# MartinPippel/DAmar

Hardware: AMD Instinct MI355X
Metric: aligned base-pairs/sec (daligner block-vs-block) (higher is better)
Workload: dtype int32

## Files before the change

### damar_amd/api.py

```python
import ctypes as C
import os

from .lib import load, bin_path

c_int64 = C.c_int64


class HITS_READ(C.Structure):
    _fields_ = [("rlen", C.c_int), ("boff", c_int64), ("coff", c_int64), ("flags", C.c_int)]


class HITS_DB(C.Structure):
    _fields_ = [("ureads", C.c_int), ("freq", C.c_float * 4), ("maxlen", C.c_int),
                ("totlen", c_int64), ("nreads", C.c_int), ("part", C.c_int), ("ufirst", C.c_int),
                ("path", C.c_char_p), ("loaded", C.c_int), ("bases", C.c_void_p),
                ("reads", C.POINTER(HITS_READ)), ("tracks", C.c_void_p)]


class SimParams(C.Structure):
    _fields_ = [("genome_mbp", C.c_double), ("coverage", C.c_double), ("bias", C.c_double),
                ("seed", C.c_int), ("rmean", C.c_int), ("rsdev", C.c_int), ("rshort", C.c_int),
                ("erate", C.c_double), ("block_mbp", C.c_int), ("min_len", C.c_int),
                ("tandem_frac", C.c_double), ("max_blocks", C.c_int)]

# ... 94 lines not shown
        L.damar_index_bytes.argtypes = [C.c_void_p]
        L.damar_index_bytes.restype = C.c_uint64
        L.damar_complement_copy.argtypes = [C.POINTER(HITS_DB), C.POINTER(HITS_DB)]
        L.damar_free_complement.argtypes = [C.POINTER(HITS_DB)]
        L.damar_async_drain.argtypes = []
        L.damar_set_bread_range.argtypes = [C.c_int, C.c_int]
        L.damar_index_download.argtypes = [C.c_void_p, C.c_void_p]
        L.damar_match.argtypes = [C.POINTER(HITS_DB), C.POINTER(HITS_DB), C.c_void_p, C.c_void_p,
                                  C.c_int, C.c_int, C.c_void_p, C.POINTER(c_int64)]
        L.damar_match_batch.argtypes = [C.POINTER(MatchJob), C.c_int]
        L.damar_set_async.argtypes = [C.c_int]
        L.damar_async_totals.argtypes = [C.POINTER(c_int64), C.POINTER(C.c_double), C.POINTER(C.c_double)]
        L.damar_async_counts.argtypes = [C.POINTER(c_int64), C.POINTER(C.c_double), C.POINTER(c_int64)]
        L.damar_wave_totals.argtypes = [C.POINTER(c_int64)] * 3
        L.damar_write_overlaps.argtypes = [C.c_void_p, C.c_char_p, C.c_char_p, C.c_char_p, C.c_char_p, C.c_int]
        L.damar_tandem_set_params.argtypes = [C.c_int] * 4
        L.damar_tandem_set_params.restype = C.c_int
        L.Match_Self.argtypes = [C.c_char_p, C.POINTER(HITS_DB), C.c_void_p]
        L.damar_match_self.argtypes = [C.POINTER(HITS_DB), C.c_void_p, C.c_void_p, C.POINTER(c_int64)]
        L.damar_last_seeds.argtypes = [C.c_void_p, c_int64]
        L.damar_last_seeds.restype = c_int64
        L.damar_order_runs_test.argtypes = [C.c_void_p, c_int64, C.c_int, C.c_int, C.c_void_p, C.c_int]
        L.damar_order_runs_test.restype = C.c_int
        L.damar_local_alignment_batch.argtypes = [C.c_void_p, C.c_void_p, C.c_int, C.c_void_p,
                                                  C.POINTER(C.c_int), C.c_int, C.POINTER(C.c_int),
                                                  C.POINTER(c_int64), C.POINTER(C.c_uint16), c_int64]
        L.damar_local_alignment_batch.restype = C.c_int
        L.damar_local_alignment_batch_opts.argtypes = L.damar_local_alignment_batch.argtypes + [C.c_int, C.POINTER(C.c_int),
                                                                                               C.POINTER(C.c_int)]
        L.damar_local_alignment_batch_opts.restype = C.c_int
        L.damar_last_timings.argtypes = [C.POINTER(C.c_double)]
        L.damar_last_counters.argtypes = [C.POINTER(c_int64)]
        L.damar_last_slabs.argtypes = [C.POINTER(C.c_int), C.POINTER(c_int64), C.c_int]
        L.damar_last_slabs.restype = C.c_int
        L.damar_slab_totals.argtypes = [C.POINTER(c_int64)]
        L.damar_slab_cut.argtypes = [C.POINTER(C.c_uint64), C.c_int, C.c_uint64, C.POINTER(C.c_int), C.POINTER(c_int64), C.c_int]
        L.damar_slab_cut.restype = C.c_int
        L.damar_bench_sort_u32.argtypes = [C.c_uint32, C.c_int, C.c_int, C.c_uint32]
        L.damar_bench_sort_u32.restype = C.c_double
        L.damar_set_check.argtypes = [C.c_int]
        L.damar_check_totals.argtypes = [C.POINTER(c_int64)]
        L.damar_check_note_blocks.argtypes = [C.c_void_p, C.POINTER(HITS_DB), C.POINTER(HITS_DB)]
        L.damar_pile_coverage.argtypes = [C.POINTER(PileBatch), C.POINTER(RepeatParams), C.POINTER(c_int64), C.POINTER(c_int64), C.POINTER(c_int64)]
        L.damar_pile_repeats.argtypes = [C.POINTER(PileBatch), C.POINTER(RepeatParams), C.POINTER(PileTrack)]
        L.damar_pile_tandem.argtypes = [C.POINTER(PileBatch), C.c_int, C.POINTER(PileTrack)]
        L.damar_pile_last.argtypes = [C.POINTER(C.c_double), C.POINTER(c_int64)]
# ... 444 lines not shown
```

### damar_amd/csrc/kernels/kernels.h

```cpp
#ifndef DAMAR_KERNELS_H
#define DAMAR_KERNELS_H

#include "dev_common.h"

size_t damar_scan_workspace_bytes(u64 n);
void   damar_exclusive_scan_u32(const u32 *in, u32 *out, u64 n, void *work, u64 *total_dev, hipStream_t st);
#define DAMAR_SCAN_TILE 4096
void   damar_tile_offsets_u32(const u32 *in, u64 n, void *work, u64 *total_dev, hipStream_t st);
void   damar_scan_tile_counts(u32 *tcount, u32 ntiles, u64 *total_dev, hipStream_t st);
size_t damar_sort_workspace_bytes(u64 n);
void   damar_sort_set_threads(int threads);
const u32 *damar_sort_error_word(const void *work);
int    damar_radix_sort_keys_u64(u64 *k0, u64 *k1, u64 n, int lobit, int hibit, void *work, hipStream_t st);
void   damar_radix_sort_split_u64(u64 *k0, u64 *k1, u64 n, int lobit, int hibit, u32 *ohi, u32 *olo, void *work,
                                  hipStream_t st);
int    damar_radix_sort_u32(u32 *k0, u32 *v0, u32 *k1, u32 *v1, u64 n, int nbits, void *work, hipStream_t st);
int    damar_radix_sort_keys_u32(u32 *k0, u32 *k1, u64 n, int nbits, void *work, hipStream_t st);
int    damar_radix_sort_u64(u64 *k0, u32 *v0, u64 *k1, u32 *v1, u64 n, int nbits, void *work, hipStream_t st);

enum { DAMAR_PILE_COVER = 0, DAMAR_PILE_REPEAT = 1, DAMAR_PILE_TANDEM = 2 };
#define DAMAR_PILE_ERR_RANGE 1u
typedef struct
{
  const long long *pile_off;
  const int *pile_aread, *abpos, *aepos, *bbpos, *bepos, *bread, *flags, *read_len, *read_flags;
  u32   npiles;
  int   mode, pbits;
  int   min_len, inc_identity, inccov, enter, leave, merge_dist;
  u64  *keys;
  u32  *kept;
  const u32 *koff;
// ... 131 lines not shown
} MergeArgs;

typedef struct { u32 b0, b1, ja, ia;
                 u32 sh, pad[3]; } MergeTile;

size_t damar_merge_workspace_bytes(u32 alen);
u32   *damar_merge_tile_counts(void *work, u32 alen);
u32    damar_merge_tiles(u32 alen);
void   damar_launch_merge_count(const MergeArgs *m, void *work, unsigned long long *gram, u32 ngram, hipStream_t st);
void damar_launch_merge_emit(const MergeArgs *m, void *work, u64 nhits, u64 *keys, u32 *vals, u32 *pid, hipStream_t st);
void damar_launch_merge_bread_hist(const MergeArgs *m, void *work, unsigned long long *hist, hipStream_t st);
void damar_launch_merge_range(const MergeArgs *m, void *work, hipStream_t st);
void damar_launch_pair_heads_ids(const u32 *pids, u64 nhits, u64 off, u64 gtotal, int abits, int minhit, int nshift,
                                 u64 *send, u64 *bits, void *scan_work, u64 *total_dev, u32 *heads, hipStream_t st);
void damar_launch_pair_bitmap(const u32 *pids, const u32 *heads, u32 nheads, int abits, u32 b_lo, u32 b_hi, u32 *bitmap,
                              hipStream_t st);
void damar_launch_seed_cut_count(const u64 *keys, u64 nhits, int pbits, const u32 *bitmap, u32 *tcount, u64 *total_dev,
                                 hipStream_t st);
void damar_launch_seed_cut_scatter(const u64 *keys, const u32 *vals, u64 nhits, int pbits, const u32 *bitmap,
                                   const u32 *toff, u64 *okeys, u32 *ovals, hipStream_t st);
void damar_launch_pair_heads(const u64 *keys, u64 nhits, u64 off, u64 gtotal, int pbits, int abits, int minhit, int nshift,
                             u64 *send , u64 *bits, void *scan_work, u64 *total_dev,
                             u32 *heads, hipStream_t st);
void damar_launch_pair_work(u64 *keys, const u32 *vals, u64 nhits, u64 off, u64 gtotal, int ppos, int dbits, int abits, int minhit, int nshift,
                            u64 *send , u64 *bits, void *scan_work, u64 *total_dev ,
                            int binshift, int kmer, int hitmin, u32 b_lo, u32 b_hi, int unsorted, hipStream_t st);
size_t damar_order_runs_scratch_bytes(u64 nhits);
void damar_launch_order_runs(u64 *keys, u64 nhits, int ppos, int dbits, const u32 *work, u32 nwork, void *scratch, hipStream_t st);
void damar_launch_pair_work_expand(const u64 *bits, const void *scan_work, u64 nhits, u32 *work, hipStream_t st);
#define WORK_COST_BITS 16
#define WORK_COST_MAX  ((1u << WORK_COST_BITS) - 1)
void damar_launch_work_cost(const u64 *keys, const u32 *vals, u64 nhits, int pbits, int abits, int dbits, const u32 *aboff,
                            const u32 *bboff, const u32 *work, u32 nwork, u32 coarse, u32 *key, u32 *val, hipStream_t st);
void damar_launch_pair_screen(const u64 *keys, const u32 *vals, u64 nhits, int pbits, int dbits, const u32 *heads, u32 nheads,
                              int minhit, int binshift, int kmer, int hitmin, int abits, u32 b_lo, u32 b_hi, u32 *keep, hipStream_t st);
void damar_launch_compact_u32(const u32 *src, const u32 *keep, const u32 *off, u32 n, u32 *out, hipStream_t st);
void damar_launch_compact_index(const u32 *flags, const u32 *off, u64 n, u32 *out, hipStream_t st);

#ifdef __HIPCC__
__device__ __forceinline__ int seed_diag(u64 k, const u32 *__restrict__ vals, u64 i, u64 pmask, int dbits)
{ if (dbits)
    return (int) ((k >> dbits) & pmask) - (int) (k & ((1ull << dbits) - 1));
  return (int) vals[i];
}
#endif

typedef struct
{ int abpos, bbpos, aepos, bepos, diffs;
  int atlen, btlen;
  int aread, bread;
  u32 item, seq;
  u32 toff;
// ... 147 lines not shown
```

### damar_amd/csrc/kernels/seed_merge.hip

```cpp
#include "dev_common.h"
#include "kernels.h"

SEED_PRIO_VAR(g_merge_prio, 0)
SEED_PRIO_SETTER(damar_merge_set_prio, g_merge_prio)


__device__ __forceinline__ u32 count_below(const u32 *__restrict__ bpos, u32 jb, u32 ib, u32 bound)
{ u32 a = jb, b = ib;
  while (a < b)
    { u32 m = (a + b) >> 1;
      if (bpos[m] < bound) a = m + 1; else b = m;
    }
  return a - jb;
}


#ifndef MT_PER
#define MT_PER  4
#endif
#define MT_A    (MT_PER * 256)
#define MT_BCAP (3 * MT_A)
#define MT_HITS 4
#define MT_NBK  2048

// ... 838 lines not shown
}

void damar_launch_merge_bread_hist(const MergeArgs *m, void *work, unsigned long long *hist, hipStream_t st)
{ if (m->alen == 0)
    return;
  const u32 ntiles = (u32) mw_tiles(m->alen);
  const u32 *cnt = (const u32 *) ((char *) work + mw_off_cnt(m->alen)), *jb = (const u32 *) ((char *) work + mw_off_jb(m->alen));
  hipLaunchKernelGGL(merge_bread_hist, dim3(ntiles), dim3(256), 0, st, *m, (const MergeTile *) work, cnt, jb, hist);
}

void damar_launch_merge_range(const MergeArgs *m, void *work, hipStream_t st)
{ if (m->alen == 0)
    return;
  const u32 ntiles = (u32) mw_tiles(m->alen);
  u32 *tcount = damar_merge_tile_counts(work, m->alen);
  u32 *cnt = (u32 *) ((char *) work + mw_off_cnt(m->alen)), *jb = (u32 *) ((char *) work + mw_off_jb(m->alen));
  hipLaunchKernelGGL(merge_range, dim3(ntiles), dim3(256), 0, st, *m, (const MergeTile *) work, tcount, cnt, jb);
}

#define SCREEN_MAX   48
#define SCREEN_PANEL 50000
template <typename K>
__global__ __launch_bounds__(64)
void slice_ends(const K *__restrict__ keys, u64 nhits, u64 off, u64 gtotal, int bshift, int nshift, u64 *__restrict__ send)
{ const int nthr = 1 << nshift, t = threadIdx.x;
  if (t >= nthr)
    return;
  const u64 g = (t == nthr - 1) ? gtotal : (gtotal * (u64) (t + 1)) >> nshift;
  u64 e;
  if (g <= off)
    e = 0;
  else if (g > off + nhits)
    e = ~0ull;
  else
    { e = g - off;
      u64 d = keys[e - 1] >> bshift, a = e, b = nhits;
      while (a < b)
        { u64 mid = (a + b) >> 1;
          if ((keys[mid] >> bshift) == d) a = mid + 1; else b = mid;
        }
      e = a;
    }
  send[t] = e;
}

#define PH_ROUNDS (DAMAR_SCAN_TILE / 256)
template <typename K>
__global__ __launch_bounds__(256)
// ... 43 lines not shown
                    for (int t = 0; t < nthr; t++)
                      { u64 e = send[t];
                        if (i < e)
                          { if (i + (u64) minhit >= e) f = false;
                            break;
                          }
                      }
                }
            }
          const u64 m = __ballot(f);
          if (l == 0)
            { bits[(base >> 6) + (u64) r * 4 + w] = m;
              mine += (u32) __popcll(m);
            }
        }
    }
  if (l == 0) wsum[w] = mine;
  __syncthreads();
  if (threadIdx.x == 0)
    tcount[blockIdx.x] = wsum[0] + wsum[1] + wsum[2] + wsum[3];
}

__global__ __launch_bounds__(64)
void pair_heads_expand(const u64 *__restrict__ bits, const u32 *__restrict__ toff, u32 *__restrict__ heads)
{ const u64 wi = (u64) blockIdx.x * 64u + threadIdx.x;
  u64 m = bits[wi];
  const int c = __popcll(m);
  u32 o = toff[blockIdx.x] + (u32) (wave_incl_scan_i(c) - c);
  const u32 first = (u32) (wi << 6);
  while (m)
    { const int b = __ffsll((long long) m) - 1;
      m &= m - 1;
      heads[o++] = first + (u32) b;
    }
}

template <typename K>
static void pair_heads_impl(const K *keys, u64 nhits, u64 off, u64 gtotal, int pbits, int abits, int minhit, int nshift,
                            u64 *send , u64 *bits, void *scan_work, u64 *total_dev,
                            u32 *heads, hipStream_t st)
{ if (nhits == 0)
    { HIP_CHECK(hipMemsetAsync(total_dev, 0, sizeof(u64), st));
      return;
    }
  if (nshift > 6)
    nshift = 6;
  const u32 ntiles = (u32) ((nhits + DAMAR_SCAN_TILE - 1) / DAMAR_SCAN_TILE);
  u32 *tcount = (u32 *) scan_work;
  if (nshift >= 0)
    hipLaunchKernelGGL(slice_ends<K>, dim3(1), dim3(64), 0, st, keys, nhits, off, gtotal, abits + pbits, nshift, send);
  hipLaunchKernelGGL(pair_heads_mark<K>, dim3(ntiles), dim3(256), 0, st, keys, nhits, pbits, minhit, nshift, send, bits, tcount);
  damar_scan_tile_counts(tcount, ntiles, total_dev, st);
  hipLaunchKernelGGL(pair_heads_expand, dim3(ntiles), dim3(64), 0, st, bits, tcount, heads);
}

void damar_launch_pair_heads(const u64 *keys, u64 nhits, u64 off, u64 gtotal, int pbits, int abits, int minhit, int nshift,
                             u64 *send, u64 *bits, void *scan_work, u64 *total_dev, u32 *heads, hipStream_t st)
{ pair_heads_impl<u64>(keys, nhits, off, gtotal, pbits, abits, minhit, nshift, send, bits, scan_work, total_dev, heads, st);
}


void damar_launch_pair_heads_ids(const u32 *pids, u64 nhits, u64 off, u64 gtotal, int abits, int minhit, int nshift,
                                 u64 *send, u64 *bits, void *scan_work, u64 *total_dev, u32 *heads, hipStream_t st)
{ pair_heads_impl<u32>(pids, nhits, off, gtotal, 0, abits, minhit, nshift, send, bits, scan_work, total_dev, heads, st);
}

__global__ __launch_bounds__(256)
void pair_bitmap_set(const u32 *__restrict__ pids, const u32 *__restrict__ heads, u32 nheads, int abits, u32 b_lo, u32 b_hi,
                     u32 *__restrict__ bitmap)
{ const u32 t = blockIdx.x * 256u + threadIdx.x;
  if (t >= nheads)
    return;
  const u32 p = pids[heads[t]], rb = p >> abits;
  if (rb < b_lo || rb >= b_hi)
    return;
  atomicOr(&bitmap[p >> 5], 1u << (p & 31));
// ... 172 lines not shown
          for (int y = 0; y < q; y++)
            prev = (d[y] == d[q]) ? c[y] : prev;
        }
      add[q] = min(c[q] - prev, kmer);
    }
  if (UNS && top > SCREEN_PANEL)
    return true;
  bool ok = false;
#pragma unroll
  for (int x = 0; x < N; x++)
    { int sum = 0;
#pragma unroll
      for (int y = 0; y < N; y++)
        sum += ((u32) (d[y] - d[x]) <= 1u) ? add[y] : 0;
      ok |= (x < n) && (sum >= hitmin);
    }
  return ok;
}

template <bool UNS>
__global__ __launch_bounds__(256)
void pair_work_mark(const u64 *__restrict__ keys, const u32 *__restrict__ vals, u64 nhits, int ppos, int dbits, int abits,
                    int minhit, int nshift, const u64 *__restrict__ send, int binshift, int kmer, int hitmin,
                    u32 b_lo, u32 b_hi, u64 *__restrict__ bits, u32 *__restrict__ tcount)
{ SEED_PRIO(g_merge_prio);
  __shared__ u64 sk[DAMAR_SCAN_TILE + PW_HALO + 1];
  __shared__ u64 bb[(PH_ROUNDS + 1) * 4];
  __shared__ u16 hl[DAMAR_SCAN_TILE];
  __shared__ u16 cl[DAMAR_SCAN_TILE];
  __shared__ u32 kb[DAMAR_SCAN_TILE / 32];
  __shared__ u32 bl[DAMAR_SCAN_TILE / PW_SMALL];
  __shared__ u32 nh, nlo, nhi, nb;
  const int  pshift = ppos + dbits;
  const u64  pmask = (1ull << ppos) - 1;
  const int  nthr = nshift < 0 ? 0 : 1 << nshift;
  const int  l = lane_id(), w = threadIdx.x >> 6;
  const u64  base = (u64) blockIdx.x * DAMAR_SCAN_TILE;
  {
    constexpr int NLD = (DAMAR_SCAN_TILE + PW_HALO + 1 + 255) / 256;
    u64 v[NLD];
#pragma unroll
    for (int q = 0; q < NLD; q++)
      { u64 i = base + (u64) q * 256u + threadIdx.x;
        i = i > 0 ? i - 1 : 0;
        v[q] = keys[i < nhits ? i : nhits - 1];
      }
#pragma unroll
// ... 180 lines not shown
        }
      int s0 = 0, s1 = 0, p0 = 0, p1 = 0;
#pragma unroll 4
      for (int y = 0; y < n; y++)
        { const u64 ky = sk[off + 1 + (u32) y];
          const int dy = seed_diag(ky, vals, i + (u64) y, pmask, dbits) >> binshift;
          const int ap = (int) ((ky >> dbits) & pmask);
          if (dy == dx)
            { s0 += (ap - p0 >= kmer) ? kmer : ap - p0;  p0 = ap; }
          else if (dy == dx + 1)
            { s1 += (ap - p1 >= kmer) ? kmer : ap - p1;  p1 = ap; }
        }
      if (__ballot(s0 + s1 >= hitmin) != 0 && l == 0)
        atomicOr(&kb[off >> 5], 1u << (off & 31));
    }
  __syncthreads();
  if (threadIdx.x < 64)
    { const u64 m = (u64) kb[2 * threadIdx.x] | ((u64) kb[2 * threadIdx.x + 1] << 32);
      bits[(base >> 6) + threadIdx.x] = m;
      const int c = wave_incl_scan_i(__popcll(m));
      if (threadIdx.x == 63)
        tcount[blockIdx.x] = (u32) c;
    }
}

#define OR_MAX   2048
#define OR_WAVE  512
#define OR_SLICE 32
__device__ __forceinline__ u32 run_length(const u64 *keys, u64 nhits, u64 i, int pshift, u32 maxrun, int l, u64 pr)
{ u32 n = 0;
  for (;;)
    { const u64 x = i + (u64) n + (u64) l;
      const u64 same = __ballot(x < nhits && (keys[x] >> pshift) == pr);
      if (same != ~0ull)
        return n + (u32) __ffsll((long long) ~same) - 1u;
      n += 64;
      if (n > maxrun)
        return n;
    }
}

__global__ __launch_bounds__(256)
void order_probe(const u64 *__restrict__ keys, u64 nhits, int ppos, int dbits, const u64 *__restrict__ bits, u64 *__restrict__ flag,
                 u32 maxrun)
{ SEED_PRIO(g_merge_prio);
  __shared__ u16 hl[DAMAR_SCAN_TILE];
  __shared__ u32 nh;
  const int  l = lane_id();
  const u64  base = (u64) blockIdx.x * DAMAR_SCAN_TILE;
  if (threadIdx.x == 0)
    nh = 0;
  __syncthreads();
  if (threadIdx.x < DAMAR_SCAN_TILE / 64)
    { u64 w = bits[(base >> 6) + threadIdx.x];
      while (w)
        { const int b = __ffsll((long long) w) - 1;
          w &= w - 1;
          hl[atomicAdd(&nh, 1u)] = (u16) (threadIdx.x * 64u + (u32) b);
        }
    }
  __syncthreads();
  const u32 n_h = nh;
  bool over = false;
  for (u32 h = threadIdx.x >> 6; h < n_h; h += 4)
    { const u64 i = base + hl[h];
      over |= run_length(keys, nhits, i, ppos + dbits, maxrun, l, keys[i] >> (ppos + dbits)) > maxrun;
    }
  if (over && l == 0)
    atomicOr((unsigned long long *) flag, 1ull);
}

template <u32 J>
__device__ __forceinline__ u32 lane_xor(u32 v)
{ if constexpr (J == 1)
    return (u32) __builtin_amdgcn_update_dpp(0, (int) v, 0xB1, 0xf, 0xf, true);
  else if constexpr (J == 2)
    return (u32) __builtin_amdgcn_update_dpp(0, (int) v, 0x4E, 0xf, 0xf, true);
  else if constexpr (J == 8)
    return (u32) __builtin_amdgcn_update_dpp(0, (int) v, 0x128, 0xf, 0xf, true);
  else if constexpr (J == 4 || J == 16)
    return (u32) __builtin_amdgcn_ds_swizzle((int) v, (int) (0x1f | (J << 10)));
  else
    return (u32) __shfl_xor((int) v, (int) J);
}

template <int K, u32 K2, u32 JJ>
__device__ __forceinline__ void or_step(u32 (&c)[K], int l)
{ if constexpr (JJ >= 64)
    {
#pragma unroll
      for (int q = 0; q < K; q++)
        if ((q & (int) (JJ >> 6)) == 0)
// ... 146 lines not shown
        keys[i + j] = rk[ck[j] & 2047u];
      __syncthreads();
    }
}

size_t damar_order_runs_scratch_bytes(u64 nhits)
{ return sizeof(u32) * (size_t) (2 * (nhits / (OR_WAVE + 1)) + 2); }

#ifdef OR_STATS
static void or_stats_print(void)
{ unsigned long long h[16];
  if (hipMemcpyFromSymbol(h, HIP_SYMBOL(g_or_hist), sizeof(h)) != hipSuccess)
    return;
  unsigned long long runs = 0;
  for (int b = 0; b <= 12; b++)
    runs += h[b];
  fprintf(stderr, "order_runs: %llu kept runs, %llu seeds in them\n", runs, h[13]);
  for (int b = 0; b <= 12; b++)
    if (h[b])
      fprintf(stderr, "  runs of %5d..%-5d %9llu  (%.3f %%)\n", b == 0 ? 1 : (1 << b) + 1, b == 12 ? 1 << 30 : 2 << b, h[b], 100. * h[b] / runs);
}
#endif

void damar_launch_order_runs(u64 *keys, u64 nhits, int ppos, int dbits, const u32 *work, u32 nwork, void *scratch, hipStream_t st)
{ if (nwork == 0)
    return;
#ifdef OR_STATS
  static int reg = 0;
  if (!reg)
    { reg = 1;  atexit(or_stats_print); }
#endif
  u32 *lcount = (u32 *) scratch;
  HIP_CHECK(hipMemsetAsync(lcount, 0, sizeof(u32), st));
  const u32 slice = std::min<u32>(OR_SLICE, 4u * std::max<u32>(1u, nwork / 2048u));
  hipLaunchKernelGGL(order_waves, dim3((nwork + slice - 1) / slice), dim3(256), 0, st, keys, nhits, ppos, dbits, work, nwork, slice,
                     lcount, lcount + 2);
  if (nhits > OR_WAVE)
    { const u64 most = nhits / (OR_WAVE + 1);
      hipLaunchKernelGGL(order_long, dim3((u32) std::min<u64>(std::min<u64>(nwork, most), 1024)), dim3(256), 0, st, keys, ppos, dbits,
                         (const u32 *) lcount, (const u32 *) (lcount + 2));
    }
}

void damar_launch_pair_work(u64 *keys, const u32 *vals, u64 nhits, u64 off, u64 gtotal, int ppos, int dbits, int abits, int minhit, int nshift,
                            u64 *send, u64 *bits, void *scan_work, u64 *total_dev, int binshift, int kmer, int hitmin,
                            u32 b_lo, u32 b_hi, int unsorted, hipStream_t st)
{ HIP_CHECK(hipMemsetAsync(total_dev, 0, 2 * sizeof(u64), st));
  if (nhits == 0)
    return;
  if (nshift > 6)
    nshift = 6;
  const u32 ntiles = (u32) ((nhits + DAMAR_SCAN_TILE - 1) / DAMAR_SCAN_TILE);
  u32 *tcount = (u32 *) scan_work;
  if (nshift >= 0)
    hipLaunchKernelGGL(slice_ends<u64>, dim3(1), dim3(64), 0, st, keys, nhits, off, gtotal, abits + ppos + dbits, nshift, send);
  if (!unsorted)
    hipLaunchKernelGGL(pair_work_mark<false>, dim3(ntiles), dim3(256), 0, st, (const u64 *) keys, vals, nhits, ppos, dbits, abits, minhit,
                       nshift, (const u64 *) send, binshift, kmer, hitmin, b_lo, b_hi, bits, tcount);
  else
    { hipLaunchKernelGGL(pair_work_mark<true>, dim3(ntiles), dim3(256), 0, st, (const u64 *) keys, vals, nhits, ppos, dbits, abits, minhit,
                         nshift, (const u64 *) send, binshift, kmer, hitmin, b_lo, b_hi, bits, tcount);
      static int maxrun = -1;
      if (maxrun < 0)
        { const char *e = getenv("DAMAR_TEST_RUN_MAX");
          maxrun = (e && atoi(e) >= 2 && atoi(e) <= OR_MAX) ? atoi(e) : OR_MAX;
        }
      hipLaunchKernelGGL(order_probe, dim3(ntiles), dim3(256), 0, st, (const u64 *) keys, nhits, ppos, dbits, (const u64 *) bits, total_dev + 1,
                         (u32) maxrun);
    }
  damar_scan_tile_counts(tcount, ntiles, total_dev, st);
}

void damar_launch_pair_work_expand(const u64 *bits, const void *scan_work, u64 nhits, u32 *work, hipStream_t st)
{ if (nhits == 0)
    return;
  const u32 ntiles = (u32) ((nhits + DAMAR_SCAN_TILE - 1) / DAMAR_SCAN_TILE);
  hipLaunchKernelGGL(pair_heads_expand, dim3(ntiles), dim3(64), 0, st, bits, (const u32 *) scan_work, work);
}

__global__ __launch_bounds__(256)
void compact_u32(const u32 *__restrict__ src, const u32 *__restrict__ keep, const u32 *__restrict__ off, u32 n,
                 u32 *__restrict__ out)
{ u32 i = blockIdx.x * 256u + threadIdx.x;
  if (i < n && keep[i])
    out[off[i]] = src[i];
}

void damar_launch_compact_u32(const u32 *src, const u32 *keep, const u32 *off, u32 n, u32 *out, hipStream_t st)
{ if (n == 0)
    return;
  hipLaunchKernelGGL(compact_u32, dim3((n + 255) / 256), dim3(256), 0, st, src, keep, off, n, out);
}

__global__ __launch_bounds__(256)
void compact_index(const u32 *__restrict__ flags, const u32 *__restrict__ off, u64 n, u32 *__restrict__ out)
{ u64 i = (u64) blockIdx.x * 256u + threadIdx.x;
  if (i < n && flags[i])
    out[off[i]] = (u32) i;
}

// ... 59 lines not shown
```

### damar_amd/csrc/kernels/sort_scan.hip

```cpp
#include "dev_common.h"
#include "kernels.h"

#define SCAN_THREADS 256
#define SCAN_ITEMS   16
#define SCAN_TILE    (SCAN_THREADS * SCAN_ITEMS)


__device__ __forceinline__ u32 block_excl_scan_256(u32 v, u32 *lds4, u32 *total)
{ int l = lane_id(), w = threadIdx.x >> 6;
  u32 inc = (u32) wave_incl_scan_i((int) v);
  if (l == 63) lds4[w] = inc;
  __syncthreads();
  u32 base = 0, tot = 0;
  for (int i = 0; i < 4; i++)
    { u32 s = lds4[i];
      if (i < w) base += s;
      tot += s;
    }
  __syncthreads();
  *total = tot;
  return base + inc - v;
}

__global__ __launch_bounds__(SCAN_THREADS)
// ... 19 lines not shown
      if (i < ntiles) tsum[i] = (u32) (carry + ex);
      carry += tot;
    }
  if (threadIdx.x == 0) *total = carry;
}

__global__ __launch_bounds__(SCAN_THREADS)
void scan_tile_apply(const u32 *__restrict__ in, u32 *__restrict__ out, u64 n, const u32 *__restrict__ toff)
{ __shared__ u32 lds4[4];
  u64 base = (u64) blockIdx.x * SCAN_TILE + (u64) threadIdx.x * SCAN_ITEMS;
  u32 v[SCAN_ITEMS], s = 0;
  for (int i = 0; i < SCAN_ITEMS; i++)
    { v[i] = (base + i < n) ? in[base + i] : 0;
      s += v[i];
    }
  u32 tot;
  u32 ex = block_excl_scan_256(s, lds4, &tot) + toff[blockIdx.x];
  for (int i = 0; i < SCAN_ITEMS; i++)
    { if (base + i < n) out[base + i] = ex;
      ex += v[i];
    }
}

size_t damar_scan_workspace_bytes(u64 n)
{ u64 ntiles = (n + SCAN_TILE - 1) / SCAN_TILE;
  return ((((size_t) (ntiles + 1) * sizeof(u32)) + 63) & ~(size_t) 63) + 64;
}

void damar_exclusive_scan_u32(const u32 *in, u32 *out, u64 n, void *work, u64 *total_dev, hipStream_t st)
{ u32 ntiles = (u32) ((n + SCAN_TILE - 1) / SCAN_TILE);
  u32 *tsum = (u32 *) work;
  if (n == 0)
    { HIP_CHECK(hipMemsetAsync(total_dev, 0, sizeof(u64), st));
      return;
    }
  hipLaunchKernelGGL(scan_tile_sums, dim3(ntiles), dim3(SCAN_THREADS), 0, st, in, n, tsum);
  hipLaunchKernelGGL(scan_tile_offsets, dim3(1), dim3(SCAN_THREADS), 0, st, tsum, ntiles, total_dev);
  hipLaunchKernelGGL(scan_tile_apply, dim3(ntiles), dim3(SCAN_THREADS), 0, st, in, out, n, tsum);
}

void damar_tile_offsets_u32(const u32 *in, u64 n, void *work, u64 *total_dev, hipStream_t st)
{ u32 ntiles = (u32) ((n + SCAN_TILE - 1) / SCAN_TILE);
  u32 *tsum = (u32 *) work;
  if (n == 0)
    { HIP_CHECK(hipMemsetAsync(total_dev, 0, sizeof(u64), st));
      return;
    }
  hipLaunchKernelGGL(scan_tile_sums, dim3(ntiles), dim3(SCAN_THREADS), 0, st, in, n, tsum);
  hipLaunchKernelGGL(scan_tile_offsets, dim3(1), dim3(SCAN_THREADS), 0, st, tsum, ntiles, total_dev);
}

void damar_scan_tile_counts(u32 *tcount, u32 ntiles, u64 *total_dev, hipStream_t st)
{ hipLaunchKernelGGL(scan_tile_offsets, dim3(1), dim3(SCAN_THREADS), 0, st, tcount, ntiles, total_dev);
}

void damar_preload_scan(void)
{ hipFuncAttributes fa;
  (void) hipFuncGetAttributes(&fa, (const void *) scan_tile_sums);
}
```

### damar_amd/csrc/shim.hip

```cpp
#include <algorithm>
#include <vector>
#include <deque>
#include <string>
#include <thread>
#include <atomic>
#include <mutex>
#include <condition_variable>
#include <functional>
#include <string.h>
#include <unistd.h>

#include "kernels/dev_common.h"
#include <ctype.h>
#include "kernels/kernels.h"

extern "C" {
#include "damar_filter.h"
#include "damar_hip.h"
#include "host/damar_host.h"
}

#define MAXGRAM 10000

static void die(void)
// ... 2197 lines not shown
  stage("run_heads");
  tick(3);
  HIP_CHECK(hipMemcpyAsync(got, s.tot, 2 * sizeof(u64), hipMemcpyDeviceToHost, G_st));
  stream_wait(G_st);
  if (s.psort && got[1] != 0)
    { G_cnt[7] += 1;
      if (s.keys == s.tk || s.resort_ws == NULL)
        { fprintf(stderr, "damar: internal error, no room to sort the seeds again\n");
          die();
        }
      const SortBufs again = { s.keys, s.tk, NULL, NULL, s.resort_ws, NULL };
      if (sort_seeds(s, again, s.total, false))
        HIP_CHECK(hipMemcpyAsync(s.keys, s.tk, sizeof(u64) * (size_t) s.total, hipMemcpyDeviceToDevice, G_st));
      damar_launch_pair_work(s.keys, s.vals, s.total, s.s_off, s.s_all, m.pbits, m.dbits, m.abits, s.minhit, s.hshift, s.sends,
                             (u64 *) s.foff, s.scw2, s.tot, P_binshift, P_kmer, P_hitmin, P_bread_lo, P_bread_hi, 0, G_st);
      HIP_CHECK(hipMemcpyAsync(got, s.tot, 2 * sizeof(u64), hipMemcpyDeviceToHost, G_st));
      stream_wait(G_st);
      s.psort = false;
    }
  const u64 nwork64 = got[0];
  arena_reserve(s.ord, work_list_bytes(nwork64));
  s.work = (u32 *) arena_take(s.ord, sizeof(u32) * ((size_t) nwork64 + 1));
  if (nwork64 > 0)
    { damar_launch_pair_work_expand((const u64 *) s.foff, s.scw2, s.total, s.work, G_st);
      if (s.psort)
        damar_launch_order_runs(s.keys, s.total, m.pbits, m.dbits, s.work, (u32) nwork64, s.order_ws, G_st);
    }
  stage("work_list");
  s.nwork = (u32) nwork64;
}

static void front_work_twostep(SeedStage &s)
{ const MergeArgs &m = s.m;
  u64 nwork64 = 0;
  u32 *heads = (u32 *) s.tk;
  damar_launch_pair_heads(s.keys, s.total, s.s_off, s.s_all, m.pbits + m.dbits, m.abits, s.minhit, s.hshift, s.sends,
                          (u64 *) s.foff , s.scw2, s.tot, heads, G_st);
  stage("run_heads");
  HIP_CHECK(hipMemcpyAsync(&nwork64, s.tot, sizeof(u64), hipMemcpyDeviceToHost, G_st));
  HIP_CHECK(hipStreamSynchronize(G_st));
  const u32 nheads = (u32) nwork64;
  arena_reserve(s.ord, work_list_bytes(nheads));
  s.work = (u32 *) arena_take(s.ord, sizeof(u32) * ((size_t) nheads + 1));
  nwork64 = 0;
  if (nheads > 0)
    { damar_launch_pair_screen(s.keys, s.vals, s.total, m.pbits, m.dbits, heads, nheads, s.minhit, P_binshift, P_kmer, P_hitmin,
                               m.abits, P_bread_lo, P_bread_hi, s.flags, G_st);
      damar_exclusive_scan_u32(s.flags, s.foff, nheads, s.scw2, s.tot, G_st);
      damar_launch_compact_u32(heads, s.flags, s.foff, nheads, s.work, G_st);
// ... 862 lines not shown
      if (hits) hits[i] = G_plan.hits[(size_t) i];
    }
  if (b_lo != NULL && n <= cap && (size_t) n < G_plan.b_lo.size())
    b_lo[n] = G_plan.b_lo[(size_t) n];
  return n;
}

extern "C" void damar_slab_totals(int64 *out)
{ out[0] = G_slab_tot[0];  out[1] = G_slab_tot[1]; }

extern "C" int damar_order_runs_test(uint64 *keys, int64 nhits, int ppos, int dbits, const uint32 *work, int nwork)
{ finish_all();
  ensure_init();
  if (nhits <= 0 || nwork <= 0)
    return 0;
  u64  *dk;
  u32  *dw;
  void *sc;
  HIP_CHECK(hipMalloc((void **) &dk, sizeof(u64) * (size_t) nhits));
  HIP_CHECK(hipMalloc((void **) &dw, sizeof(u32) * (size_t) nwork));
  HIP_CHECK(hipMalloc(&sc, damar_order_runs_scratch_bytes((u64) nhits)));
  HIP_CHECK(hipMemcpy(dk, keys, sizeof(u64) * (size_t) nhits, hipMemcpyHostToDevice));
  HIP_CHECK(hipMemcpy(dw, work, sizeof(u32) * (size_t) nwork, hipMemcpyHostToDevice));
  damar_launch_order_runs(dk, (u64) nhits, ppos, dbits, dw, (u32) nwork, sc, G_st);
  HIP_CHECK(hipStreamSynchronize(G_st));
  HIP_CHECK(hipMemcpy(keys, dk, sizeof(u64) * (size_t) nhits, hipMemcpyDeviceToHost));
  HIP_CHECK(hipFree(dk));  HIP_CHECK(hipFree(dw));  HIP_CHECK(hipFree(sc));
  return 0;
}

extern "C" int64 damar_last_seeds(void *out, int64 cap)
{ struct SP { int diag, apos, aread, bread; } *sp = (SP *) out;
  if (out == NULL)
    { G_keep_seeds = (cap != 0);
      return 0;
    }
  int64 n = (int64) G_seed_keys.size();
  for (int64 i = 0; i < n && i < cap; i++)
    { u64 k = G_seed_keys[(size_t) i];
      const int bpos = (int) (k & ((1ull << G_seed_dbits) - 1));
      k >>= G_seed_dbits;
      sp[i].apos  = (int) (k & ((1ull << G_seed_pbits) - 1));
      sp[i].aread = (int) ((k >> G_seed_pbits) & ((1ull << G_seed_abits) - 1));
      sp[i].bread = (int) (k >> (G_seed_pbits + G_seed_abits));
      sp[i].diag  = G_seed_dbits ? sp[i].apos - bpos : (int) G_seed_vals[(size_t) i];
    }
  return n;
}

extern "C" int damar_local_alignment_batch_opts(damar_dev_block *ablk, damar_dev_block *bblk, int comp,
// ... 942 lines not shown
```

### include/damar_hip.h

```cpp
#ifndef DAMAR_HIP_H
#define DAMAR_HIP_H

#include "damar_db.h"
#include "damar_align.h"

#ifdef __cplusplus
extern "C" {
#endif

int   damar_hip_init(int device);
int   damar_hip_numa_node(int device);
const char *damar_hip_device_name(void);
void  damar_hip_sync(void);
void  damar_prewarm(int gigabytes);

typedef struct damar_dev_block damar_dev_block;
damar_dev_block *damar_block_upload(const HITS_DB *block);
void damar_block_preload(const HITS_DB *block);
damar_dev_block *damar_block_upload_bg(const HITS_DB *block);
damar_dev_block *damar_block_upload_packed(const HITS_DB *block, const damar_packed *pk, int comp);
void             damar_packed_forget(const HITS_DB *block);
void             damar_block_free(damar_dev_block *blk);

typedef struct damar_dev_index damar_dev_index;
// ... 17 lines not shown
  Align_Spec *spec;
  int64 counts[3];
} damar_match_job;
void damar_match_batch(damar_match_job *jobs, int njobs);

void damar_set_bread_range(int lo, int hi);

void damar_set_async(int on);
void damar_async_drain(void);
void damar_async_totals(int64 *ncheck, double *tail_ms, double *write_ms);
void damar_async_counts(int64 *seed_hits, double *report_ms, int64 *launches);
double damar_async_d2h_ms(void);
void damar_wave_totals(int64 *cells, int64 *half_steps, int64 *iterations);
void damar_write_overlaps(Align_Spec *spec, const char *dirName1, const char *dirName2,
                          const char *ablock, const char *bblock, int lastRead);

int  damar_tandem_set_params(int kmer, int binshift, int hitmin, int nthreads);
void damar_match_self(const HITS_DB *ablock, damar_dev_block *blk, Align_Spec *spec, int64 *counts);
void Match_Self(char *aname, HITS_DB *ablock, Align_Spec *settings);

int64 damar_last_seeds(void *out, int64 cap);

int damar_order_runs_test(uint64 *keys, int64 nhits, int ppos, int dbits, const uint32 *work, int nwork);

int  damar_last_slabs(int *b_lo , int64 *hits , int cap);
void damar_slab_totals(int64 *out );
int  damar_slab_cut(const uint64_t *hits, int nreads, uint64_t cap, int *b_lo , int64 *sums ,
                    int max_slabs);

int damar_last_limit(void);

void damar_bias_reset(void);

int damar_local_alignment_batch(damar_dev_block *ablk, damar_dev_block *bblk, int comp,
                                Align_Spec *spec, const int *tasks, int ntasks,
                                int *paths, int64 *trace_off, uint16 *traces, int64 trace_cap);
int damar_local_alignment_batch_opts(damar_dev_block *ablk, damar_dev_block *bblk, int comp,
                                     Align_Spec *spec, const int *tasks, int ntasks,
                                     int *paths, int64 *trace_off, uint16 *traces, int64 trace_cap,
                                     int t8, int *t8_fell_back, int *wide_tasks);

int  damar_trace_pts(damar_dev_block *ablk, int afirst, damar_dev_block *bblk, int bfirst,
                     const Overlap *ovls, int64 novl, int tbytes, int tspace, int mode, int same,
                     int64 *soff, int *diffs, int **script);
int  damar_trace_mid(damar_dev_block *ablk, int afirst, damar_dev_block *bblk, int bfirst,
                     const Overlap *ovls, int64 novl, int tbytes, int tspace, int mode, int same,
// ... 71 lines not shown
```

Before: 53.88 billion.

## Cut launches in pair-work stage: fold probe, memsets, and scan into fewer kernels

Folds the separate order_probe kernel into pair_work_mark, which now checks the run-length limit from shared memory and sets the overflow flag. Replaces hipMemsetAsync calls with zeroing done inside existing kernels (slice_ends, pair_heads_expand). Adds a single-block exclusive scan for small inputs so the multi-kernel tile scan is skipped. The goal is less launch and memset overhead in the seed pipeline. The risks are extra work in the mark kernel and correctness that now depends on the order in which the zeroing happens.

After: 54.03 billion (median of 2 runs). Within noise of the previous version (+0.3%).

```diff
diff --git a/damar_amd/api.py b/damar_amd/api.py
--- a/damar_amd/api.py
+++ b/damar_amd/api.py
@@ -140,6 +140,10 @@
         L.damar_last_seeds.restype = c_int64
         L.damar_order_runs_test.argtypes = [C.c_void_p, c_int64, C.c_int, C.c_int, C.c_void_p, C.c_int]
         L.damar_order_runs_test.restype = C.c_int
+        L.damar_scan_test.argtypes = [C.c_void_p, C.c_void_p, c_int64, C.c_void_p, C.c_int, C.c_int]
+        L.damar_scan_test.restype = C.c_int
+        L.damar_pair_work_test.argtypes = [C.c_void_p, c_int64] + [C.c_int] * 8 + [C.c_void_p, C.c_void_p]
+        L.damar_pair_work_test.restype = C.c_int
         L.damar_local_alignment_batch.argtypes = [C.c_void_p, C.c_void_p, C.c_int, C.c_void_p,
                                                   C.POINTER(C.c_int), C.c_int, C.POINTER(C.c_int),
                                                   C.POINTER(c_int64), C.POINTER(C.c_uint16), c_int64]
diff --git a/damar_amd/csrc/kernels/kernels.h b/damar_amd/csrc/kernels/kernels.h
--- a/damar_amd/csrc/kernels/kernels.h
+++ b/damar_amd/csrc/kernels/kernels.h
@@ -6,7 +6,6 @@
 size_t damar_scan_workspace_bytes(u64 n);
 void   damar_exclusive_scan_u32(const u32 *in, u32 *out, u64 n, void *work, u64 *total_dev, hipStream_t st);
 #define DAMAR_SCAN_TILE 4096
-void   damar_tile_offsets_u32(const u32 *in, u64 n, void *work, u64 *total_dev, hipStream_t st);
 void   damar_scan_tile_counts(u32 *tcount, u32 ntiles, u64 *total_dev, hipStream_t st);
 size_t damar_sort_workspace_bytes(u64 n);
 void   damar_sort_set_threads(int threads);
@@ -184,12 +183,15 @@
 void damar_launch_pair_heads(const u64 *keys, u64 nhits, u64 off, u64 gtotal, int pbits, int abits, int minhit, int nshift,
                              u64 *send , u64 *bits, void *scan_work, u64 *total_dev,
                              u32 *heads, hipStream_t st);
+void damar_pair_work_set_run_max(int maxrun);
 void damar_launch_pair_work(u64 *keys, const u32 *vals, u64 nhits, u64 off, u64 gtotal, int ppos, int dbits, int abits, int minhit, int nshift,
                             u64 *send , u64 *bits, void *scan_work, u64 *total_dev ,
                             int binshift, int kmer, int hitmin, u32 b_lo, u32 b_hi, int unsorted, hipStream_t st);
 size_t damar_order_runs_scratch_bytes(u64 nhits);
-void damar_launch_order_runs(u64 *keys, u64 nhits, int ppos, int dbits, const u32 *work, u32 nwork, void *scratch, hipStream_t st);
-void damar_launch_pair_work_expand(const u64 *bits, const void *scan_work, u64 nhits, u32 *work, hipStream_t st);
+void damar_launch_order_runs(u64 *keys, u64 nhits, int ppos, int dbits, const u32 *work, u32 nwork, void *scratch, int cleared,
+                             hipStream_t st);
+void damar_launch_pair_work_expand(const u64 *bits, const void *scan_work, u64 nhits, u32 *work, void *order_scratch ,
+                                   hipStream_t st);
 #define WORK_COST_BITS 16
 #define WORK_COST_MAX  ((1u << WORK_COST_BITS) - 1)
 void damar_launch_work_cost(const u64 *keys, const u32 *vals, u64 nhits, int pbits, int abits, int dbits, const u32 *aboff,
diff --git a/damar_amd/csrc/kernels/seed_merge.hip b/damar_amd/csrc/kernels/seed_merge.hip
--- a/damar_amd/csrc/kernels/seed_merge.hip
+++ b/damar_amd/csrc/kernels/seed_merge.hip
@@ -884,8 +884,11 @@
 #define SCREEN_PANEL 50000
 template <typename K>
 __global__ __launch_bounds__(64)
-void slice_ends(const K *__restrict__ keys, u64 nhits, u64 off, u64 gtotal, int bshift, int nshift, u64 *__restrict__ send)
+void slice_ends(const K *__restrict__ keys, u64 nhits, u64 off, u64 gtotal, int bshift, int nshift, u64 *__restrict__ send,
+                u64 *__restrict__ zero )
 { const int nthr = 1 << nshift, t = threadIdx.x;
+  if (t == 0 && zero != NULL)
+    *zero = 0;
   if (t >= nthr)
     return;
   const u64 g = (t == nthr - 1) ? gtotal : (gtotal * (u64) (t + 1)) >> nshift;
@@ -975,8 +978,11 @@
 }
 
 __global__ __launch_bounds__(64)
-void pair_heads_expand(const u64 *__restrict__ bits, const u32 *__restrict__ toff, u32 *__restrict__ heads)
+void pair_heads_expand(const u64 *__restrict__ bits, const u32 *__restrict__ toff, u32 *__restrict__ heads,
+                       u32 *__restrict__ zero )
 { const u64 wi = (u64) blockIdx.x * 64u + threadIdx.x;
+  if (wi == 0 && zero != NULL)
+    *zero = 0;
   u64 m = bits[wi];
   const int c = __popcll(m);
   u32 o = toff[blockIdx.x] + (u32) (wave_incl_scan_i(c) - c);
@@ -1001,10 +1007,10 @@
   const u32 ntiles = (u32) ((nhits + DAMAR_SCAN_TILE - 1) / DAMAR_SCAN_TILE);
   u32 *tcount = (u32 *) scan_work;
   if (nshift >= 0)
-    hipLaunchKernelGGL(slice_ends<K>, dim3(1), dim3(64), 0, st, keys, nhits, off, gtotal, abits + pbits, nshift, send);
+    hipLaunchKernelGGL(slice_ends<K>, dim3(1), dim3(64), 0, st, keys, nhits, off, gtotal, abits + pbits, nshift, send, (u64 *) NULL);
   hipLaunchKernelGGL(pair_heads_mark<K>, dim3(ntiles), dim3(256), 0, st, keys, nhits, pbits, minhit, nshift, send, bits, tcount);
   damar_scan_tile_counts(tcount, ntiles, total_dev, st);
-  hipLaunchKernelGGL(pair_heads_expand, dim3(ntiles), dim3(64), 0, st, bits, tcount, heads);
+  hipLaunchKernelGGL(pair_heads_expand, dim3(ntiles), dim3(64), 0, st, bits, tcount, heads, (u32 *) NULL);
 }
 
 void damar_launch_pair_heads(const u64 *keys, u64 nhits, u64 off, u64 gtotal, int pbits, int abits, int minhit, int nshift,
@@ -1223,7 +1229,8 @@
 __global__ __launch_bounds__(256)
 void pair_work_mark(const u64 *__restrict__ keys, const u32 *__restrict__ vals, u64 nhits, int ppos, int dbits, int abits,
                     int minhit, int nshift, const u64 *__restrict__ send, int binshift, int kmer, int hitmin,
-                    u32 b_lo, u32 b_hi, u64 *__restrict__ bits, u32 *__restrict__ tcount)
+                    u32 b_lo, u32 b_hi, u64 *__restrict__ bits, u32 *__restrict__ tcount,
+                    u64 *__restrict__ toolong , u32 maxrun)
 { SEED_PRIO(g_merge_prio);
   __shared__ u64 sk[DAMAR_SCAN_TILE + PW_HALO + 1];
   __shared__ u64 bb[(PH_ROUNDS + 1) * 4];
@@ -1450,6 +1457,22 @@
       if (threadIdx.x == 63)
         tcount[blockIdx.x] = (u32) c;
     }
+  if (UNS)
+    { bool over = false;
+      u32 m = (kb[threadIdx.x >> 1] >> ((threadIdx.x & 1u) << 4)) & 0xffffu;
+      while (m)
+        { const u32 off = (threadIdx.x << 4) + (u32) (__ffs((int) m) - 1);
+          m &= m - 1;
+          const u64 x = base + off + maxrun;
+          if (x < nhits)
+            { const u32 j = off + 1 + maxrun;
+              const u64 kx = (j < DAMAR_SCAN_TILE + PW_HALO + 1) ? sk[j] : keys[x];
+              over |= (kx >> pshift) == (sk[off + 1] >> pshift);
+            }
+        }
+      if (__syncthreads_or(over) && threadIdx.x == 0)
+        atomicOr((unsigned long long *) toolong, 1ull);
+    }
 }
 
 #define OR_MAX   2048
@@ -1466,36 +1489,6 @@
       if (n > maxrun)
         return n;
     }
-}
-
-__global__ __launch_bounds__(256)
-void order_probe(const u64 *__restrict__ keys, u64 nhits, int ppos, int dbits, const u64 *__restrict__ bits, u64 *__restrict__ flag,
-                 u32 maxrun)
-{ SEED_PRIO(g_merge_prio);
-  __shared__ u16 hl[DAMAR_SCAN_TILE];
-  __shared__ u32 nh;
-  const int  l = lane_id();
-  const u64  base = (u64) blockIdx.x * DAMAR_SCAN_TILE;
-  if (threadIdx.x == 0)
-    nh = 0;
-  __syncthreads();
-  if (threadIdx.x < DAMAR_SCAN_TILE / 64)
-    { u64 w = bits[(base >> 6) + threadIdx.x];
-      while (w)
-        { const int b = __ffsll((long long) w) - 1;
-          w &= w - 1;
-          hl[atomicAdd(&nh, 1u)] = (u16) (threadIdx.x * 64u + (u32) b);
-        }
-    }
-  __syncthreads();
-  const u32 n_h = nh;
-  bool over = false;
-  for (u32 h = threadIdx.x >> 6; h < n_h; h += 4)
-    { const u64 i = base + hl[h];
-      over |= run_length(keys, nhits, i, ppos + dbits, maxrun, l, keys[i] >> (ppos + dbits)) > maxrun;
-    }
-  if (over && l == 0)
-    atomicOr((unsigned long long *) flag, 1ull);
 }
 
 template <u32 J>
@@ -1688,7 +1681,8 @@
 }
 #endif
 
-void damar_launch_order_runs(u64 *keys, u64 nhits, int ppos, int dbits, const u32 *work, u32 nwork, void *scratch, hipStream_t st)
+void damar_launch_order_runs(u64 *keys, u64 nhits, int ppos, int dbits, const u32 *work, u32 nwork, void *scratch, int cleared,
+                             hipStream_t st)
 { if (nwork == 0)
     return;
 #ifdef OR_STATS
@@ -1697,7 +1691,8 @@
     { reg = 1;  atexit(or_stats_print); }
 #endif
   u32 *lcount = (u32 *) scratch;
-  HIP_CHECK(hipMemsetAsync(lcount, 0, sizeof(u32), st));
+  if (!cleared)
+    HIP_CHECK(hipMemsetAsync(lcount, 0, sizeof(u32), st));
   const u32 slice = std::min<u32>(OR_SLICE, 4u * std::max<u32>(1u, nwork / 2048u));
   hipLaunchKernelGGL(order_waves, dim3((nwork + slice - 1) / slice), dim3(256), 0, st, keys, nhits, ppos, dbits, work, nwork, slice,
                      lcount, lcount + 2);
@@ -1708,10 +1703,15 @@
     }
 }
 
+static int G_test_run_max = 0;
+void damar_pair_work_set_run_max(int maxrun) { G_test_run_max = (maxrun >= 2 && maxrun <= OR_MAX) ? maxrun : 0; }
+
 void damar_launch_pair_work(u64 *keys, const u32 *vals, u64 nhits, u64 off, u64 gtotal, int ppos, int dbits, int abits, int minhit, int nshift,
                             u64 *send, u64 *bits, void *scan_work, u64 *total_dev, int binshift, int kmer, int hitmin,
                             u32 b_lo, u32 b_hi, int unsorted, hipStream_t st)
-{ HIP_CHECK(hipMemsetAsync(total_dev, 0, 2 * sizeof(u64), st));
+{
+  if (nhits == 0 || nshift < 0)
+    HIP_CHECK(hipMemsetAsync(total_dev, 0, 2 * sizeof(u64), st));
   if (nhits == 0)
     return;
   if (nshift > 6)
@@ -1719,29 +1719,29 @@
   const u32 ntiles = (u32) ((nhits + DAMAR_SCAN_TILE - 1) / DAMAR_SCAN_TILE);
   u32 *tcount = (u32 *) scan_work;
   if (nshift >= 0)
-    hipLaunchKernelGGL(slice_ends<u64>, dim3(1), dim3(64), 0, st, keys, nhits, off, gtotal, abits + ppos + dbits, nshift, send);
+    hipLaunchKernelGGL(slice_ends<u64>, dim3(1), dim3(64), 0, st, keys, nhits, off, gtotal, abits + ppos + dbits, nshift, send,
+                       total_dev + 1);
   if (!unsorted)
     hipLaunchKernelGGL(pair_work_mark<false>, dim3(ntiles), dim3(256), 0, st, (const u64 *) keys, vals, nhits, ppos, dbits, abits, minhit,
-                       nshift, (const u64 *) send, binshift, kmer, hitmin, b_lo, b_hi, bits, tcount);
+                       nshift, (const u64 *) send, binshift, kmer, hitmin, b_lo, b_hi, bits, tcount, (u64 *) NULL, 0u);
   else
-    { hipLaunchKernelGGL(pair_work_mark<true>, dim3(ntiles), dim3(256), 0, st, (const u64 *) keys, vals, nhits, ppos, dbits, abits, minhit,
-                         nshift, (const u64 *) send, binshift, kmer, hitmin, b_lo, b_hi, bits, tcount);
-      static int maxrun = -1;
-      if (maxrun < 0)
+    { static int envrun = -1;
+      if (envrun < 0)
         { const char *e = getenv("DAMAR_TEST_RUN_MAX");
-          maxrun = (e && atoi(e) >= 2 && atoi(e) <= OR_MAX) ? atoi(e) : OR_MAX;
-        }
-      hipLaunchKernelGGL(order_probe, dim3(ntiles), dim3(256), 0, st, (const u64 *) keys, nhits, ppos, dbits, (const u64 *) bits, total_dev + 1,
-                         (u32) maxrun);
+          envrun = (e && atoi(e) >= 2 && atoi(e) <= OR_MAX) ? atoi(e) : OR_MAX;
+        }
+      const int maxrun = G_test_run_max ? G_test_run_max : envrun;
+      hipLaunchKernelGGL(pair_work_mark<true>, dim3(ntiles), dim3(256), 0, st, (const u64 *) keys, vals, nhits, ppos, dbits, abits, minhit,
+                         nshift, (const u64 *) send, binshift, kmer, hitmin, b_lo, b_hi, bits, tcount, total_dev + 1, (u32) maxrun);
     }
   damar_scan_tile_counts(tcount, ntiles, total_dev, st);
 }
 
-void damar_launch_pair_work_expand(const u64 *bits, const void *scan_work, u64 nhits, u32 *work, hipStream_t st)
+void damar_launch_pair_work_expand(const u64 *bits, const void *scan_work, u64 nhits, u32 *work, void *order_scratch, hipStream_t st)
 { if (nhits == 0)
     return;
   const u32 ntiles = (u32) ((nhits + DAMAR_SCAN_TILE - 1) / DAMAR_SCAN_TILE);
-  hipLaunchKernelGGL(pair_heads_expand, dim3(ntiles), dim3(64), 0, st, bits, (const u32 *) scan_work, work);
+  hipLaunchKernelGGL(pair_heads_expand, dim3(ntiles), dim3(64), 0, st, bits, (const u32 *) scan_work, work, (u32 *) order_scratch);
 }
 
 __global__ __launch_bounds__(256)
diff --git a/damar_amd/csrc/kernels/sort_scan.hip b/damar_amd/csrc/kernels/sort_scan.hip
--- a/damar_amd/csrc/kernels/sort_scan.hip
+++ b/damar_amd/csrc/kernels/sort_scan.hip
@@ -65,6 +65,90 @@
     }
 }
 
+#define SCAN1_THREADS 1024
+#define SCAN1_ITEMS   16
+#define SCAN1_SPAN    (SCAN1_THREADS * SCAN1_ITEMS)
+#define SCAN1_MAX     (2 * SCAN1_SPAN)
+
+__device__ __forceinline__ void scan1_load(const u32 *in, u64 n, u64 at, u32 (&v)[SCAN1_ITEMS])
+{ if (at + SCAN1_ITEMS <= n)
+    {
+#pragma unroll
+      for (int q = 0; q < SCAN1_ITEMS / 4; q++)
+        { const uint4 x = ((const uint4 *) (in + at))[q];
+          v[4 * q] = x.x;  v[4 * q + 1] = x.y;  v[4 * q + 2] = x.z;  v[4 * q + 3] = x.w;
+        }
+    }
+  else
+    {
+#pragma unroll
+      for (int i = 0; i < SCAN1_ITEMS; i++)
+        v[i] = (at + i < n) ? in[at + i] : 0u;
+    }
+}
+
+__global__ __launch_bounds__(SCAN1_THREADS)
+void scan_one_launch(const u32 *in, u32 *out, u64 n, u64 *__restrict__ total)
+{ __shared__ u64 wsum[SCAN1_THREADS / 64];
+  const int l = lane_id(), w = threadIdx.x >> 6;
+  u64 carry = 0;
+  u32 nx[SCAN1_ITEMS];
+  scan1_load(in, n, (u64) threadIdx.x * SCAN1_ITEMS, nx);
+  for (u64 b = 0; b < n; b += SCAN1_SPAN)
+    { const u64 at = b + (u64) threadIdx.x * SCAN1_ITEMS;
+      u32 v[SCAN1_ITEMS];
+      u64 s = 0;
+#pragma unroll
+      for (int i = 0; i < SCAN1_ITEMS; i++)
+        { v[i] = nx[i];
+          s += v[i];
+        }
+      if (b + SCAN1_SPAN < n)
+        scan1_load(in, n, at + SCAN1_SPAN, nx);
+      u64 inc = s;
+      for (int o = 1; o < 64; o <<= 1)
+        { const u64 t = __shfl_up(inc, o);
+          if (l >= o) inc += t;
+        }
+      if (l == 63) wsum[w] = inc;
+      __syncthreads();
+      u64 before = 0, tot = 0;
+#pragma unroll
+      for (int i = 0; i < SCAN1_THREADS / 64; i++)
+        { const u64 x = wsum[i];
+          if (i < w) before += x;
+          tot += x;
+        }
+      __syncthreads();
+      u64 ex = carry + before + inc - s;
+      if (at + SCAN1_ITEMS <= n)
+        {
+#pragma unroll
+          for (int q = 0; q < SCAN1_ITEMS / 4; q++)
+            { uint4 x;
+              x.x = (u32) ex;  ex += v[4 * q];
+              x.y = (u32) ex;  ex += v[4 * q + 1];
+              x.z = (u32) ex;  ex += v[4 * q + 2];
+              x.w = (u32) ex;  ex += v[4 * q + 3];
+              ((uint4 *) (out + at))[q] = x;
+            }
+        }
+      else
+        {
+#pragma unroll
+          for (int i = 0; i < SCAN1_ITEMS; i++)
+            { if (at + i < n) out[at + i] = (u32) ex;
+              ex += v[i];
+            }
+        }
+      carry += tot;
+    }
+  if (threadIdx.x == 0) *total = carry;
+}
+
+static bool scan_one_fits(const void *in, const void *out, u64 n)
+{ return n <= SCAN1_MAX && (((uintptr_t) in | (uintptr_t) out) & 15u) == 0; }
+
 size_t damar_scan_workspace_bytes(u64 n)
 { u64 ntiles = (n + SCAN_TILE - 1) / SCAN_TILE;
   return ((((size_t) (ntiles + 1) * sizeof(u32)) + 63) & ~(size_t) 63) + 64;
@@ -73,8 +157,8 @@
 void damar_exclusive_scan_u32(const u32 *in, u32 *out, u64 n, void *work, u64 *total_dev, hipStream_t st)
 { u32 ntiles = (u32) ((n + SCAN_TILE - 1) / SCAN_TILE);
   u32 *tsum = (u32 *) work;
-  if (n == 0)
-    { HIP_CHECK(hipMemsetAsync(total_dev, 0, sizeof(u64), st));
+  if (scan_one_fits(in, out, n))
+    { hipLaunchKernelGGL(scan_one_launch, dim3(1), dim3(SCAN1_THREADS), 0, st, in, out, n, total_dev);
       return;
     }
   hipLaunchKernelGGL(scan_tile_sums, dim3(ntiles), dim3(SCAN_THREADS), 0, st, in, n, tsum);
@@ -82,19 +166,11 @@
   hipLaunchKernelGGL(scan_tile_apply, dim3(ntiles), dim3(SCAN_THREADS), 0, st, in, out, n, tsum);
 }
 
-void damar_tile_offsets_u32(const u32 *in, u64 n, void *work, u64 *total_dev, hipStream_t st)
-{ u32 ntiles = (u32) ((n + SCAN_TILE - 1) / SCAN_TILE);
-  u32 *tsum = (u32 *) work;
-  if (n == 0)
-    { HIP_CHECK(hipMemsetAsync(total_dev, 0, sizeof(u64), st));
-      return;
-    }
-  hipLaunchKernelGGL(scan_tile_sums, dim3(ntiles), dim3(SCAN_THREADS), 0, st, in, n, tsum);
-  hipLaunchKernelGGL(scan_tile_offsets, dim3(1), dim3(SCAN_THREADS), 0, st, tsum, ntiles, total_dev);
-}
-
 void damar_scan_tile_counts(u32 *tcount, u32 ntiles, u64 *total_dev, hipStream_t st)
-{ hipLaunchKernelGGL(scan_tile_offsets, dim3(1), dim3(SCAN_THREADS), 0, st, tcount, ntiles, total_dev);
+{ if (scan_one_fits(tcount, tcount, ntiles))
+    hipLaunchKernelGGL(scan_one_launch, dim3(1), dim3(SCAN1_THREADS), 0, st, (const u32 *) tcount, tcount, (u64) ntiles, total_dev);
+  else
+    hipLaunchKernelGGL(scan_tile_offsets, dim3(1), dim3(SCAN_THREADS), 0, st, tcount, ntiles, total_dev);
 }
 
 void damar_preload_scan(void)
diff --git a/damar_amd/csrc/shim.hip b/damar_amd/csrc/shim.hip
--- a/damar_amd/csrc/shim.hip
+++ b/damar_amd/csrc/shim.hip
@@ -2243,9 +2243,9 @@
   arena_reserve(s.ord, work_list_bytes(nwork64));
   s.work = (u32 *) arena_take(s.ord, sizeof(u32) * ((size_t) nwork64 + 1));
   if (nwork64 > 0)
-    { damar_launch_pair_work_expand((const u64 *) s.foff, s.scw2, s.total, s.work, G_st);
+    { damar_launch_pair_work_expand((const u64 *) s.foff, s.scw2, s.total, s.work, s.psort ? s.order_ws : NULL, G_st);
       if (s.psort)
-        damar_launch_order_runs(s.keys, s.total, m.pbits, m.dbits, s.work, (u32) nwork64, s.order_ws, G_st);
+        damar_launch_order_runs(s.keys, s.total, m.pbits, m.dbits, s.work, (u32) nwork64, s.order_ws, 1, G_st);
     }
   stage("work_list");
   s.nwork = (u32) nwork64;
@@ -3154,10 +3154,66 @@
   HIP_CHECK(hipMalloc(&sc, damar_order_runs_scratch_bytes((u64) nhits)));
   HIP_CHECK(hipMemcpy(dk, keys, sizeof(u64) * (size_t) nhits, hipMemcpyHostToDevice));
   HIP_CHECK(hipMemcpy(dw, work, sizeof(u32) * (size_t) nwork, hipMemcpyHostToDevice));
-  damar_launch_order_runs(dk, (u64) nhits, ppos, dbits, dw, (u32) nwork, sc, G_st);
+  damar_launch_order_runs(dk, (u64) nhits, ppos, dbits, dw, (u32) nwork, sc, 0, G_st);
   HIP_CHECK(hipStreamSynchronize(G_st));
   HIP_CHECK(hipMemcpy(keys, dk, sizeof(u64) * (size_t) nhits, hipMemcpyDeviceToHost));
   HIP_CHECK(hipFree(dk));  HIP_CHECK(hipFree(dw));  HIP_CHECK(hipFree(sc));
+  return 0;
+}
+
+extern "C" int damar_scan_test(const uint32 *in, uint32 *out, int64 n, uint64 *total, int reps, int inplace)
+{ finish_all();
+  ensure_init();
+  u32  *din, *dout;
+  u64  *dtot;
+  void *ws;
+  const size_t bytes = sizeof(u32) * (size_t) (n > 0 ? n : 1), wbytes = damar_scan_workspace_bytes((u64) n);
+  HIP_CHECK(hipMalloc((void **) &din, bytes));
+  HIP_CHECK(hipMalloc((void **) &dout, bytes));
+  HIP_CHECK(hipMalloc((void **) &dtot, 64));
+  HIP_CHECK(hipMalloc(&ws, wbytes));
+  HIP_CHECK(hipMemset(ws, 0xff, wbytes));
+  HIP_CHECK(hipMemset(dtot, 0xff, 64));
+  HIP_CHECK(hipMemset(dout, 0xff, bytes));
+  if (n > 0)
+    HIP_CHECK(hipMemcpy(din, in, sizeof(u32) * (size_t) n, hipMemcpyHostToDevice));
+  for (int r = 0; r < reps; r++)
+    { if (inplace && n > 0)
+        HIP_CHECK(hipMemcpyAsync(dout, din, sizeof(u32) * (size_t) n, hipMemcpyDeviceToDevice, G_st));
+      damar_exclusive_scan_u32(inplace ? dout : din, dout, (u64) n, ws, dtot, G_st);
+    }
+  HIP_CHECK(hipStreamSynchronize(G_st));
+  if (n > 0)
+    HIP_CHECK(hipMemcpy(out, dout, sizeof(u32) * (size_t) n, hipMemcpyDeviceToHost));
+  HIP_CHECK(hipMemcpy(total, dtot, sizeof(u64), hipMemcpyDeviceToHost));
+  HIP_CHECK(hipFree(din));  HIP_CHECK(hipFree(dout));  HIP_CHECK(hipFree(dtot));  HIP_CHECK(hipFree(ws));
+  return 0;
+}
+
+extern "C" int damar_pair_work_test(const uint64 *keys, int64 nhits, int ppos, int dbits, int abits, int minhit, int binshift,
+                                    int kmer, int hitmin, int maxrun, uint64 *bits, uint64 *tot)
+{ finish_all();
+  ensure_init();
+  if (nhits <= 0)
+    return 1;
+  u64  *dk, *db, *dt, *snd;
+  void *scw;
+  const size_t bbytes = bit_words_bytes((u64) nhits);
+  HIP_CHECK(hipMalloc((void **) &dk, sizeof(u64) * (size_t) nhits));
+  HIP_CHECK(hipMalloc((void **) &db, bbytes));
+  HIP_CHECK(hipMalloc((void **) &dt, 64));
+  HIP_CHECK(hipMalloc((void **) &snd, 64 * sizeof(u64)));
+  HIP_CHECK(hipMalloc(&scw, damar_scan_workspace_bytes((u64) nhits)));
+  HIP_CHECK(hipMemcpy(dk, keys, sizeof(u64) * (size_t) nhits, hipMemcpyHostToDevice));
+  HIP_CHECK(hipMemset(dt, 0xff, 64));
+  damar_pair_work_set_run_max(maxrun);
+  damar_launch_pair_work(dk, NULL, (u64) nhits, 0, (u64) nhits, ppos, dbits, abits, minhit, 0, snd, db, scw, dt, binshift, kmer, hitmin,
+                         0u, 0xffffffffu, 1, G_st);
+  damar_pair_work_set_run_max(0);
+  HIP_CHECK(hipStreamSynchronize(G_st));
+  HIP_CHECK(hipMemcpy(bits, db, bbytes, hipMemcpyDeviceToHost));
+  HIP_CHECK(hipMemcpy(tot, dt, 2 * sizeof(u64), hipMemcpyDeviceToHost));
+  HIP_CHECK(hipFree(dk));  HIP_CHECK(hipFree(db));  HIP_CHECK(hipFree(dt));  HIP_CHECK(hipFree(snd));  HIP_CHECK(hipFree(scw));
   return 0;
 }
 
diff --git a/include/damar_hip.h b/include/damar_hip.h
--- a/include/damar_hip.h
+++ b/include/damar_hip.h
@@ -63,6 +63,11 @@
 int64 damar_last_seeds(void *out, int64 cap);
 
 int damar_order_runs_test(uint64 *keys, int64 nhits, int ppos, int dbits, const uint32 *work, int nwork);
+
+int damar_scan_test(const uint32 *in, uint32 *out, int64 n, uint64 *total, int reps, int inplace);
+
+int damar_pair_work_test(const uint64 *keys, int64 nhits, int ppos, int dbits, int abits, int minhit, int binshift,
+                         int kmer, int hitmin, int maxrun, uint64 *bits, uint64 *tot);
 
 int  damar_last_slabs(int *b_lo , int64 *hits , int cap);
 void damar_slab_totals(int64 *out );
```
